# haoyuzhao123/CGRayTracing

Hardware: AMD Instinct MI355X
Metric: Mrays/sec (primary+secondary) at 1920x1080 spp=64 (higher is better)
Workload: dtype f64

## Files before the change

cgraytracing_amd/_capi.py:

```python
from __future__ import annotations

import ctypes as C
import os

import sys

_HERE = os.path.dirname(os.path.abspath(__file__))
CGRT_VERSION = 112
LIB_PATH = os.path.join(_HERE, "libcgrt.so")
if os.environ.get("CGRT_LIB"):
    if os.environ.get("CGRT_DEV_LIBS") == "1":
        LIB_PATH = os.environ["CGRT_LIB"]
        print("cgraytracing_amd: DEVELOPMENT library %s (CGRT_LIB + CGRT_DEV_LIBS=1)" % LIB_PATH, file=sys.stderr)
    else:
        print("cgraytracing_amd: CGRT_LIB ignored (set CGRT_DEV_LIBS=1 to load a development build)", file=sys.stderr)

CGRT_OK = 0
CGRT_NCOUNTERS = 8
CNT_RAYS, CNT_HITPOINTS, CNT_WAVE_ITERS, CNT_NODE_TESTS, CNT_TRI_TESTS = 0, 1, 2, 3, 4


class CgrtError(RuntimeError):
    def __init__(self, code, msg):
        super().__init__("libcgrt error %d: %s" % (code, msg))
# ... 8 lines not shown
class Grid(C.Structure):
    _fields_ = [("width", C.c_int32), ("height", C.c_int32), ("rows", C.c_int32), ("row_offset", C.c_int32),
                ("stripe_rows", C.c_int32), ("stripe_rank", C.c_int32), ("stripe_nranks", C.c_int32),
                ("spp", C.c_int32), ("sample_offset", C.c_int32), ("spp_total", C.c_int32),
                ("max_depth", C.c_int32), ("flags", C.c_int32), ("seed", C.c_uint64)]


GRID_STATS, GRID_ACCUMULATE, GRID_SPLIT_SAMPLES, GRID_NO_REORDER, GRID_FORCE_REORDER, GRID_HITPOINTS = 1, 2, 4, 8, 16, 32
GRID_NO_TILE_ORDER, GRID_DIFFUSE_TILES, GRID_NO_SPHERE_PAIRS, GRID_NO_SPHERE_MASKS = 64, 128, 256, 512
GRID_SAMPLE_RELAY, GRID_NO_SAMPLE_RELAY, GRID_SAMPLE_RELAY_4 = 1024, 2048, 4096
GRID_RELAY_MIRROR, GRID_RELAY_NO_MIRROR = 8192, 16384
GRID_RELAY_CHUNKS_FIRST, GRID_RELAY_MIRROR_FIRST, GRID_RELAY_INTERLEAVED, GRID_RELAY_ORDER_MASK = 32768, 65536, 98304, 98304
GRID_NO_LENS_STAGE, GRID_NO_SURE_TILES = 131072, 262144
GRID_RELAY_COST_START, GRID_NO_RELAY_COST_START, GRID_RELAY_BOOST, GRID_NO_RELAY_BOOST = 524288, 1048576, 2097152, 4194304
GRID_NO_LENS_TABLE, GRID_LENS_TABLE = 8388608, 16777216


class Photons(C.Structure):
    _fields_ = [("light", C.c_double * 3), ("jitter", C.c_double), ("power", C.c_double), ("alpha", C.c_double),
                ("nphotons", C.c_int64), ("hashsize", C.c_int32), ("batch", C.c_int32), ("seed", C.c_uint64),
                ("initial_radius", C.c_double), ("pair_cap", C.c_int64)]


class PpmResult(C.Structure):
    _fields_ = [("image", C.c_void_p), ("rgb8", C.c_void_p), ("hp16", C.c_void_p), ("hp_cap", C.c_uint64),
                ("hp_count", C.c_uint64), ("n_events", C.c_uint64), ("n_pairs", C.c_uint64), ("n_batch_halvings", C.c_uint64),
                ("ms_eye", C.c_double),
                ("ms_table", C.c_double), ("ms_photons", C.c_double), ("ms_gather", C.c_double)]


# ... 58 lines not shown
class RayPixels(C.Structure):
    _fields_ = [("width", C.c_int32), ("rows", C.c_int32), ("spp", C.c_int32), ("pad_", C.c_int32), ("pixel", C.c_void_p)]


class PhotonRays(C.Structure):
    _fields_ = [("n", C.c_int64), ("org3", C.c_void_p), ("dir3", C.c_void_p), ("flux3", C.c_void_p), ("keys", C.c_void_p),
                ("draws", C.c_void_p)]


RAYS_STATS = 1
RAYS_NO_SIGN_PASS = 2
RAYS_HITPOINTS = 4
RAYS_SKIP_TRANSPARENT = 8
STEP_NONE, STEP_HITPOINT, STEP_REFLECT, STEP_SPLIT = 0, 1, 2, 3
PROBE_SQRT, PROBE_NORMALIZED, PROBE_SPHERE_LEN, PROBE_SPHERE_LEN_PAIR = 0, 1, 2, 4

_DP = C.POINTER(C.c_double)
SIGNATURES = {
    "cgrt_version": (C.c_int, []),
    "cgrt_last_error": (C.c_char_p, []),
    "cgrt_scene_create": (C.c_int, [C.POINTER(C.c_void_p)]),
    "cgrt_scene_destroy": (None, [C.c_void_p]),
    "cgrt_scene_set_build": (C.c_int, [C.c_void_p, C.c_int]),
    "cgrt_scene_build_info": (C.c_int, [C.c_void_p, C.POINTER(BuildInfo)]),
    "cgrt_scene_add_sphere": (C.c_int, [C.c_void_p, _DP, C.c_double, _DP, C.c_double, C.c_double]),
    "cgrt_scene_add_texture": (C.c_int, [C.c_void_p, C.c_void_p, C.c_int, C.c_int, _DP, _DP, C.c_double,
                                         C.c_double, C.c_int]),
    "cgrt_scene_add_plane": (C.c_int, [C.c_void_p, _DP, _DP, _DP, C.c_double, C.c_double, C.c_int]),
    "cgrt_scene_add_mesh_file": (C.c_int, [C.c_void_p, C.c_char_p, C.c_double, _DP, _DP, C.c_double, C.c_double,
                                           C.c_int]),
# ... 72 lines not shown
    "cgrt_occlusion_rays_host": (C.c_int, [C.c_void_p, C.POINTER(Rays), C.POINTER(Occlusion), C.c_void_p]),
    "cgrt_occlusion_rays_variant": (C.c_int, [C.c_void_p, C.POINTER(Rays), C.c_char_p, C.c_size_t]),
    "cgrt_bounce_rays": (C.c_int, [C.c_void_p, C.POINTER(Rays), C.POINTER(Bounce), C.c_void_p, C.c_void_p]),
    "cgrt_bounce_rays_host": (C.c_int, [C.c_void_p, C.POINTER(Rays), C.POINTER(Bounce), C.c_void_p]),
    "cgrt_bounce_rays_variant": (C.c_int, [C.c_void_p, C.POINTER(Rays), C.c_char_p, C.c_size_t]),
    "cgrt_wavefront_rays": (C.c_int, [C.c_void_p, C.POINTER(Rays), C.POINTER(Wavefront), C.c_void_p, C.POINTER(C.c_uint64), C.c_void_p]),
    "cgrt_wavefront_rays_host": (C.c_int, [C.c_void_p, C.POINTER(Rays), C.POINTER(Wavefront), C.c_void_p, C.POINTER(C.c_uint64)]),
    "cgrt_wavefront_rays_variant": (C.c_int, [C.c_void_p, C.POINTER(Rays), C.c_char_p, C.c_size_t]),
    "cgrt_scene_last_wavefront": (C.c_int, [C.c_void_p, C.POINTER(C.c_int64), C.POINTER(C.c_int64), C.POINTER(C.c_int32)]),
    "cgrt_scene_last_wavefront_rays": (C.c_int, [C.c_void_p, C.c_void_p]),
    "cgrt_camera_rays": (C.c_int, [C.POINTER(Camera), C.POINTER(Grid), C.c_void_p, C.c_void_p, C.c_void_p, C.c_void_p]),
    "cgrt_camera_rays_host": (C.c_int, [C.POINTER(Camera), C.POINTER(Grid), C.c_void_p, C.c_void_p, C.c_void_p]),
    "cgrt_intersect_rays": (C.c_int, [C.c_void_p, C.c_int, C.c_void_p, C.c_void_p, C.c_void_p, C.c_int,
                                      C.c_void_p, C.c_void_p, C.c_void_p]),
    "cgrt_math_probe": (C.c_int, [C.c_int, C.c_int, C.c_void_p, C.c_int64, C.c_void_p]),
}

_lib = None


def lib():
    global _lib
    if _lib is None:
        if not os.path.exists(LIB_PATH):
            raise ImportError(
                "cgraytracing_amd: %s not found -- build the HIP library first "
                "(make -C cgraytracing_amd/csrc, or __graft_entry__.build()). There is no CPU fallback." % LIB_PATH)
        try:
            import torch
        except ImportError:
# ... 18 lines not shown
```

cgraytracing_amd/csrc/cgrt_build.cpp:

```cpp
#include "cgrt_build.h"

#include <algorithm>
#include <atomic>
#include <chrono>
#include <future>
#include <thread>
#include <unordered_map>
#include <cmath>
#include <cstdio>
#include <cstdlib>
#include <cstring>

namespace cgrt {

namespace {

inline double hi3(double a, double b, double c) { return (a > b && a > c) ? a : (b > c ? b : c); }
inline double lo3(double a, double b, double c) { return (a < b && a < c) ? a : (b < c ? b : c); }
inline float round_down(double v) {
    float f = (float)v;
    return ((double)f > v) ? std::nextafterf(f, -INFINITY) : f;
}
inline float round_up(double v) {
    float f = (float)v;
// ... 987 lines not shown
    d.light_hf_only = plane_trees ? 1 : 0;
    for (const ObjRec &o : objs)
        if (o.kind == KIND_PLANE && o.tree >= 0 && !(o.transp < kEps && trees[(size_t)o.tree].hfield >= 0)) d.light_hf_only = 0;
    d.prun_begin = d.prun_end = 0;
    if (!k.no_plane_run) {
        auto eligible = [&](int j) { return objs[(size_t)j].kind == KIND_PLANE && objs[(size_t)j].axis >= 0 && objs[(size_t)j].tree < 0; };
        int b = 0;
        while (b < d.n_lds && objs[(size_t)b].kind == KIND_PLANE && !eligible(b)) b++;
        int j = b;
        while (j < d.n_lds && eligible(j)) j++;
        if (j - b >= 3) {
            d.prun_begin = b;
            d.prun_end = j;
        }
    }
}

}
```

cgraytracing_amd/csrc/cgrt_eye.hpp:

```cpp
#ifndef CGRT_EYE_HPP
#define CGRT_EYE_HPP
#include "cgrt_lens_stage.h"
#include "cgrt_scene_walk.hpp"
#include "cgrt_sphere_mask.h"
#include "cgrt_sure_first.h"
#include "cgrt_variants.h"

struct Pending {
    V3 o, d, adj;
    int32_t depth_left;
    uint32_t path;
};

#ifndef CGRT_DIFF_WAVES
#define CGRT_DIFF_WAVES 8
#endif
#ifndef CGRT_DIFF_DOF_WAVES
#define CGRT_DIFF_DOF_WAVES 6
#endif
static constexpr int kDiffWaves = CGRT_DIFF_WAVES, kDiffDofWaves = CGRT_DIFF_DOF_WAVES;

__host__ __device__ __forceinline__ void lens_disc(uint64_t k_smp, double &sx, double &sy) {
    uint64_t ctr = k_smp;
    while (true) {
// ... 1293 lines not shown
        out[i] = sqrt_cr(in[i]);
    } else if (op == CGRT_PROBE_NORMALIZED) {
        const V3 v = normalized(ld3(in + 3 * i));
        out[3 * i] = v.x;
        out[3 * i + 1] = v.y;
        out[3 * i + 2] = v.z;
    } else if (op == CGRT_PROBE_SPHERE_LEN) {
        const double *p = in + 10 * i;
        out[i] = sphere_len(ld3(p), p[3], ld3(p + 4), ld3(p + 7));
    } else {
        const double *p = in + 14 * i;
        sphere_len_pair(ld3(p), p[3], ld3(p + 4), p[7], ld3(p + 8), ld3(p + 11), out[2 * i], out[2 * i + 1]);
    }
}

#endif
```

cgraytracing_amd/csrc/cgrt_frame.h:

```cpp
#ifndef CGRT_FRAME_H
#define CGRT_FRAME_H
#include <algorithm>
#include <cmath>
#include <cstddef>
#include <cstdint>
#include <cstdio>
#include <cstdlib>
#include <string>

#include "../../include/cgrt.h"
#include "cgrt_lens_stage.h"
#include "cgrt_relay.h"

struct GridParams {
    int32_t W, H, rows, row_offset, stripe_rows, stripe_rank, stripe_nranks;
    int32_t spp, sample_offset, max_depth;
    int32_t accumulate;
    int32_t xcd_tiles;
    int32_t chunks, chunk_spp;
    double *partial;
    uint32_t *partial_nhit;
    const unsigned char *light;
    int32_t light_mode, tile_order;
    const uint32_t *wmask;
// ... 155 lines not shown
    bool no_sure_tiles = false;
    bool no_order_reuse = false;
    int relay_chunks = kRelayDefaultChunks;
    long long relay_tiles = 0;
    int relay_mirror = -1;
    int relay_order = -1;
    int relay_start = -1;
    int relay_probe_spp = kRelayProbeSpp;
    bool relay_boost_off = false;
    uint32_t relay_boost_num = kRelayBoostNum, relay_boost_den = kRelayBoostDen;
    long long relay_boost_tiles = -1;
    int lens_stage = -1;
    int lens_table = -1;
    long long lens_table_bytes = 0;
    bool lens_table_bytes_set = false;
    const char *timeline_file = nullptr;
};
inline const char *env_str(const char *name) { const char *e = std::getenv(name); return e ? e : ""; }
inline bool env_on(const char *name) { const char *e = env_str(name); return *e && *e != '0'; }
inline int env_positive(const char *name, int def) { const int v = std::atoi(env_str(name)); return v > 0 ? v : def; }
inline int relay_order_named(const char *e) {
    const std::string v(e);
    if (v == "chunks_first" || v == "0") return kRelayChunksFirst;
    if (v == "mirror_first" || v == "1") return kRelayMirrorFirst;
    if (v == "interleaved" || v == "2") return kRelayInterleaved;
    return -1;
}
inline int relay_start_named(const char *e) {
    const std::string v(e);
    if (v == "list" || v == "0") return kRelayStartList;
// ... 59 lines not shown
            std::fprintf(stderr, "cgrt: CGRT_RELAY_START=%s names no start order of this library (list, cost): the default is used\n", env_str("CGRT_RELAY_START"));
        {
            const int ps = std::atoi(env_str("CGRT_RELAY_PROBE_SPP"));
            if (ps == 1 || ps == 2 || ps == 4) k.relay_probe_spp = ps;
        }
        k.lens_stage = lens_stage_named(env_str("CGRT_LENS_STAGE"));
        if (k.lens_stage < 0 && *env_str("CGRT_LENS_STAGE"))
            std::fprintf(stderr, "cgrt: CGRT_LENS_STAGE=%s names no form of this library (off, lds): the default is used\n", env_str("CGRT_LENS_STAGE"));
        k.lens_table = lens_table_named(env_str("CGRT_LENS_TABLE"));
        if (k.lens_table < 0 && *env_str("CGRT_LENS_TABLE"))
            std::fprintf(stderr, "cgrt: CGRT_LENS_TABLE=%s is neither off nor on: the default is used\n", env_str("CGRT_LENS_TABLE"));
        if (*env_str("CGRT_LENS_TABLE_BYTES")) {
            k.lens_table_bytes = std::max(std::atoll(env_str("CGRT_LENS_TABLE_BYTES")), 0ll);
            k.lens_table_bytes_set = true;
        }
        return k;
    }();
    EyeKnobs k = once;
    k.timeline_file = *env_str("CGRT_TIMELINE_FILE") ? env_str("CGRT_TIMELINE_FILE") : nullptr;
    if (!relay_boost_named(env_str("CGRT_RELAY_BOOST"), k.relay_boost_off, k.relay_boost_num, k.relay_boost_den)) {
        static bool said = false;
        if (!said)
            std::fprintf(stderr, "cgrt: CGRT_RELAY_BOOST=%s is neither off nor a threshold num/den (integers, num <= %u, 1 <= den <= %u): the default is used\n",
                         env_str("CGRT_RELAY_BOOST"), kRelayBoostMaxTerm, kRelayBoostMaxTerm);
        said = true;
    }
    if (*env_str("CGRT_RELAY_BOOST_TILES")) k.relay_boost_tiles = std::max(std::atoll(env_str("CGRT_RELAY_BOOST_TILES")), 0ll);
    return k;
}

// ... 284 lines not shown
```

cgraytracing_amd/csrc/cgrt_hip.hip:

```cpp
#include <hip/hip_runtime.h>

#include <algorithm>
#include <atomic>
#include <chrono>
#include <cmath>
#include <cstdio>
#include <cstdlib>
#include <cstring>
#include <exception>
#include <map>
#include <mutex>
#include <string>
#include <type_traits>
#include <vector>

#include "../../include/cgrt.h"
#include "cgrt_build.h"
#include "cgrt_rng.hpp"
#include "cgrt_types.h"

#include "cgrt_device_math.hpp"
#include "cgrt_grid.hpp"
#include "cgrt_traverse.hpp"
#include "cgrt_bezier.hpp"
// ... 605 lines not shown

enum class EyeForm { Image, Sched, SpillSph, SpillGen, Capture, Light, LightHF, Diffuse };
struct EyeLaunch {
    EyeForm form;
    EyeFlags k;
    DeviceScene dev;
    size_t lds;
    const char *what() const {
        static const char *const names[] = {"eye pass", "eye pass", "eye pass, SPILL (spheres)", "eye pass, SPILL (general)",
                                            "Hitpoint capture", "eye pass, light tiles", "eye pass, light tiles (HFONLY)",
                                            "eye pass, diffuse tiles"};
        return form <= EyeForm::Sched && k.bez ? "eye pass (Bezier)" : names[(int)form];
    }
};

static EyeLaunch eye_launch(const cgrt_scene *s, const cgrt_camera *cam, const cgrt_grid *grid, const EyeKnobs &kn, bool capture) {
    const DeviceScene &d = s->dev;
    const bool dof = cam->lens_radius > 0, glass = d.has_glass != 0 && grid->max_depth > 1;
    const bool spill = d.n_objs > d.n_lds;
    EyeLaunch L;
    L.dev = d;
    if (capture || (spill && !d.all_spheres)) {
        L.form = capture ? EyeForm::Capture : EyeForm::SpillGen;
        L.dev = with_resident(d, general_resident(s, dof, capture));
        L.k = general_flags(dof, capture, L.dev.n_objs > L.dev.n_lds);
    } else if (spill) {
        L.form = EyeForm::SpillSph;
        L.k = spill_sph_flags(dof, glass);
    } else {
        const bool bez = d.has_bezier != 0, trees = d.has_mesh != 0 || bez;
        L.k = image_flags(trees, bez, dof, glass, !trees && d.all_spheres != 0,
                          (grid->flags & CGRT_GRID_STATS) != 0 && d.has_mesh != 0 && !bez);
        const bool plain_scene = (d.has_mesh == 0 && d.has_bezier == 0) || d.single_ray != 0;
        const size_t n_wt = (size_t)((grid->width + kWaveTileW - 1) / kWaveTileW) * ((grid->rows + kWaveTileH - 1) / kWaveTileH);
        const bool reorder = grid->spp >= 4 && !(grid->flags & CGRT_GRID_NO_REORDER) && n_wt > 1 && n_wt < (1u << 30) &&
                             (!plain_scene || (grid->flags & CGRT_GRID_FORCE_REORDER) || kn.force_reorder);
        L.form = reorder ? EyeForm::Sched : EyeForm::Image;
        L.k.pair = L.form == EyeForm::Image && L.k.sph && L.k.glass && !L.k.stats && s->order.ok && !(grid->flags & CGRT_GRID_NO_SPHERE_PAIRS);
    }
    L.lds = eye_lds(L.k, L.dev) + (L.form == EyeForm::Image || L.form == EyeForm::Sched ? (size_t)kn.lds_pad : 0);
    return L;
}
static EyeLaunch light_launch(const DeviceScene &d, bool dof, const EyeKnobs &kn) {
    const bool trees = d.light_trees != 0, hf = trees && d.light_hf_only && !kn.no_hfonly;
    EyeLaunch L;
    L.form = hf ? EyeForm::LightHF : EyeForm::Light;
    L.k = light_flags(trees, dof, hf);
    L.dev = d;
    L.lds = eye_lds(L.k, d);
    return L;
}
static EyeLaunch diffuse_launch(const DeviceScene &d, bool dof) {
    EyeLaunch L;
    L.form = EyeForm::Diffuse;
// ... 286 lines not shown
int cgrt_scene_last_inkernel_diffuse_tiles(const cgrt_scene *s, int64_t *n_tiles) {
    NEED_COMMITTED(s, n_tiles);
    ON_DEVICE(s->device);
    return last_class3_tiles(s->order, TileOrderPlan::InKernel, n_tiles);
}
int cgrt_scene_last_lens_stage(const cgrt_scene *s, int64_t *lds_tiles, int64_t *area_tiles) {
    NEED_COMMITTED(s, lds_tiles && area_tiles);
    ON_DEVICE(s->device);
    return last_lens_stage(s->order, lds_tiles, area_tiles);
}
int cgrt_scene_last_lens_table(const cgrt_scene *s, int64_t *entries, int64_t *capacity, int32_t *reused) {
    NEED_COMMITTED(s, entries && capacity && reused);
    ON_DEVICE(s->device);
    return last_lens_table(s->order, s->lens, entries, capacity, reused);
}
int cgrt_scene_last_sample_relay(const cgrt_scene *s, int64_t *tiles, int32_t *chunks, int64_t *parked_values) {
    NEED_COMMITTED(s, tiles && chunks && parked_values);
    ON_DEVICE(s->device);
    return last_sample_relay(s->order, s->relay, tiles, chunks, parked_values);
}
int cgrt_scene_last_relay_form(const cgrt_scene *s, int32_t *mirror, int32_t *order) {
    NEED_COMMITTED(s, mirror && order);
    last_relay_form(s->order, s->relay, mirror, order);
    return CGRT_OK;
}

int cgrt_scene_last_relay_start(const cgrt_scene *s, uint32_t *start, int64_t start_cap, uint32_t *wcost, int64_t cost_cap, int64_t *t,
                                int64_t *n_wave_tiles, int32_t *reused) {
    NEED_COMMITTED(s, t && n_wave_tiles && reused);
    ON_DEVICE(s->device);
// ... 231 lines not shown
    if (n < 0) return fail(CGRT_ERR_INVALID, "cgrt_math_probe: negative n");
    if (n > ((int64_t)1 << 28)) return fail(CGRT_ERR_LIMIT, "cgrt_math_probe: more than 2^28 elements");
    if (n == 0) return CGRT_OK;
    const size_t n_in = op == CGRT_PROBE_SQRT ? 1 : (op == CGRT_PROBE_NORMALIZED ? 3 : (op == CGRT_PROBE_SPHERE_LEN ? 10 : 14)),
                 n_out = op == CGRT_PROBE_NORMALIZED ? 3 : (op == CGRT_PROBE_SPHERE_LEN_PAIR ? 2 : 1);
    ON_DEVICE(device);
    HostStage hs;
    const double *d_in = hs.in(in, (size_t)n * n_in * sizeof(double));
    double *d_out = hs.out(out, (size_t)n * n_out * sizeof(double));
    if (const int rc = hs.error()) return rc;
    hipLaunchKernelGGL(math_probe_kernel, dim3((unsigned)((n + 255) / 256)), dim3(256), 0, 0, op, d_in, (long long)n, d_out);
    HIP_TRY(hipGetLastError());
    return hs.finish(CGRT_OK);
}

}

#include "cgrt_ppm_plan.h"
#include "cgrt_ppm_table.hpp"
#include "cgrt_photon_trace.hpp"
#include "cgrt_ppm_apply.hpp"
#include "cgrt_ppm_session.hpp"
#include "cgrt_output.hpp"

#ifdef CGRT_UTIL
extern "C" void cgrt_util_dump(unsigned long long *out) {
    (void)hipDeviceSynchronize();
    (void)hipMemcpyFromSymbol(out, HIP_SYMBOL(g_util), sizeof(unsigned long long) * 64);
    unsigned long long z[64] = {0};
    (void)hipMemcpyToSymbol(HIP_SYMBOL(g_util), z, sizeof(z));
// ... 3 lines not shown
```

cgraytracing_amd/csrc/cgrt_scene_walk.hpp:

```cpp
#ifndef CGRT_SCENE_WALK_HPP
#define CGRT_SCENE_WALK_HPP
#include "cgrt_bezier.hpp"
#include "cgrt_traverse.hpp"
#include "cgrt_wg_lds.h"

__device__ __forceinline__ bool texture_color(const TexRec &t, const uint8_t *__restrict__ texels, V3 point, V3 &out) {
    V3 d = point - ld3(t.p);
    const V3 n = ld3(t.n);
    d = d - n * dot(d, n);
    const double te = 1e-2;
    const int rows = t.rows, cols = t.cols;
    int r, c;
    if (d.x < te && d.x > -te) {
        if (!(0 < d.y && d.y < t.lenx && 0 < d.z && d.z < t.leny)) return false;
        r = (int)floor(d.y / t.lenx * rows);
        c = (int)floor(d.z / t.leny * cols);
    } else if (d.y < te && d.y > -te) {
        if (!(0 < d.x && d.x < t.lenx && 0 < d.z && d.z < t.leny)) return false;
        c = (int)floor(d.x / t.lenx * cols);
        r = (int)floor(d.z / t.leny * rows);
    } else if (d.z < te && d.z > -te) {
        if (!(0 < d.x && d.x < t.lenx && 0 < d.y && d.y < t.leny)) return false;
        c = (int)floor(d.x / t.lenx * cols);
        r = rows - 1 - (int)floor(d.y / t.leny * rows);
// ... 249 lines not shown
        static_assert(!PAIR || (SPH && !SPILL), "PAIR: the LDS-resident sphere loop");
        static_assert(!MASKED || (SPH && !SPILL && !PAIR && !NRM), "MASKED: the terminal-diffuse body's sphere loop");
        if (MASKED && masked) {
            for (uint32_t m = mask; m != 0u; m &= m - 1u) {
                const int i = __builtin_ctz(m);
                const double len = sphere_len(objs[i], o, d);
                if (len < best.t) {
                    best.t = len;
                    best.id = i;
                }
            }
            return best;
        }
        int i_single = 0;
        if (PAIR) {
            for (int i = 0; i + 1 < n_lds; i += 2) {
                double lenA, lenB;
                const ObjRec &A = objs[i], &B = objs[i + 1];
                sphere_len_pair(ld3(A.a), A.s0, ld3(B.a), B.s0, o, d, lenA, lenB);
                if (lenA < best.t) {
                    best.t = lenA;
                    best.id = i;
                }
                if (lenB < best.t) {
                    best.t = lenB;
                    best.id = i + 1;
                }
            }
            i_single = n_lds & ~1;
        }
// ... 148 lines not shown
```

cgraytracing_amd/csrc/cgrt_types.h:

```cpp
#ifndef CGRT_TYPES_H
#define CGRT_TYPES_H
#include <stddef.h>
#include <stdint.h>

namespace cgrt {

static constexpr double kEps = 1e-4;
static constexpr double kInf = 1e10;
static constexpr int kMinKd = 10;
static constexpr double kBoxPad = 1.001e-4;
static constexpr int kMaxDepth = 5;

enum ObjKind : int32_t { KIND_SPHERE = 0, KIND_PLANE = 1, KIND_MESH = 2, KIND_BEZIER = 3 };

struct ObjRec {
    double a[3];
    double b[3];
    double s0;
    double col[3];
    double refl, transp;
    int32_t kind;
    int32_t tree;
    int32_t tex;
    int32_t aux;
// ... 115 lines not shown
    int32_t prim_obj;
    int32_t has_mesh;
    int32_t has_bezier;
    int32_t all_spheres;
    int32_t has_glass;
    int32_t cached_tree;
    int32_t cached_nodes;
    int32_t has_wide;
    int32_t light_trees;
    int32_t light_ok;
    int32_t n_cover;
    int32_t prim_finish;
    int32_t prun_begin, prun_end;
    int32_t single_ray;
    int32_t light_hf_only;
};

}
#endif
```

cgraytracing_amd/engine.py:

```python
from __future__ import annotations

import ctypes as C
import os
import weakref

import numpy as np

from . import _capi
from ._capi import Camera as _CCamera
from ._capi import Grid as _CGrid
from ._capi import check
from .scene import Camera


def _d3(v):
    return (C.c_double * 3)(*[float(x) for x in v])


_RELAY_ORDERS = ("chunks_first", "mirror_first", "interleaved")
_RELAY_STARTS = ("list", "cost")


def _grid_flags(stats, split_samples, reorder, force_reorder, tile_order, diffuse_tiles, sphere_pairs, sphere_masks, lens_stage, sure_tiles, lens_table=None):
    on = (stats, _capi.GRID_STATS), (split_samples, _capi.GRID_SPLIT_SAMPLES), (force_reorder, _capi.GRID_FORCE_REORDER), (diffuse_tiles, _capi.GRID_DIFFUSE_TILES)
    off = ((reorder, _capi.GRID_NO_REORDER), (tile_order, _capi.GRID_NO_TILE_ORDER), (sphere_pairs, _capi.GRID_NO_SPHERE_PAIRS),
           (sphere_masks, _capi.GRID_NO_SPHERE_MASKS), (lens_stage, _capi.GRID_NO_LENS_STAGE), (sure_tiles, _capi.GRID_NO_SURE_TILES))
    table = 0 if lens_table is None else _capi.GRID_LENS_TABLE if lens_table else _capi.GRID_NO_LENS_TABLE
    return sum(f for v, f in on if v) | sum(f for v, f in off if not v) | table


def _relay_flag(sample_relay, relay_mirror=None, relay_order=None, relay_start=None, relay_boost=None):
    form = 0 if relay_mirror is None else (_capi.GRID_RELAY_MIRROR if relay_mirror else _capi.GRID_RELAY_NO_MIRROR)
    if relay_boost is not None:
        form |= _capi.GRID_RELAY_BOOST if relay_boost else _capi.GRID_NO_RELAY_BOOST
    if relay_start is not None:
        if relay_start not in _RELAY_STARTS:
            raise ValueError("relay_start: None, " + ", ".join(repr(o) for o in _RELAY_STARTS))
        form |= _capi.GRID_RELAY_COST_START if relay_start == "cost" else _capi.GRID_NO_RELAY_COST_START
    if relay_order is not None:
        if relay_order not in _RELAY_ORDERS:
            raise ValueError("relay_order: None, " + ", ".join(repr(o) for o in _RELAY_ORDERS))
# ... 153 lines not shown
        return box[: n.value], ref[: n.value], need.value

    def _structs(self, camera, width, height, rows, spp, max_depth, seed, row_offset, stripe, sample_offset,
                 spp_total, flags):
        camera = camera or Camera()
        cc = _CCamera(_d3(camera.cam), camera.half_width, camera.focus_plane, camera.lens_radius)
        s_rows, s_rank, s_n = stripe if stripe else (0, 0, 1)
        g = _CGrid(width, height, rows, row_offset, s_rows, s_rank, s_n, spp, sample_offset,
                   spp_total if spp_total else spp, max_depth, flags, seed)
        return cc, g

    def trace_grid(self, width, height, spp=1, camera=None, max_depth=5, seed=12345, rows=None, row_offset=0,
                   stripe=None, sample_offset=0, spp_total=None, out=None, nhit=None, counters=None, stream=None,
                   stats=False, accumulate=False, split_samples=False, reorder=True, force_reorder=False, tile_order=True,
                   diffuse_tiles=False, sphere_pairs=True, sphere_masks=True, sample_relay=None,
                   relay_mirror=None, relay_order=None, lens_stage=True, sure_tiles=True, relay_start=None, relay_boost=None, lens_table=None):
        import torch

        rows = height - row_offset if rows is None else rows
        dev = torch.device("cuda", self.device)
        if out is None:
            out = torch.zeros((rows, width, 3), dtype=torch.float32, device=dev)
        if nhit is None:
            nhit = torch.zeros((rows, width), dtype=torch.int32, device=dev)
        elif nhit is False:
            nhit = None
        if counters is None:
            counters = torch.zeros((_capi.CGRT_NCOUNTERS,), dtype=torch.int64, device=dev)
        assert out.is_contiguous() and out.dtype == torch.float32 and tuple(out.shape) == (rows, width, 3)
        cc, g = self._structs(camera, width, height, rows, spp, max_depth, seed, row_offset, stripe, sample_offset,
                              spp_total, (_capi.GRID_ACCUMULATE if accumulate else 0) |
                              _grid_flags(stats, split_samples, reorder, force_reorder, tile_order, diffuse_tiles, sphere_pairs, sphere_masks, lens_stage, sure_tiles, lens_table) |
                              _relay_flag(sample_relay, relay_mirror, relay_order, relay_start, relay_boost))
        st = stream if stream is not None else torch.cuda.current_stream(dev).cuda_stream
        check(self._L.cgrt_trace_grid(self._h, C.byref(cc), C.byref(g), out.data_ptr(),
                                      nhit.data_ptr() if nhit is not None else None,
                                      counters.data_ptr(), C.c_void_p(st)))
        return out, nhit, counters

    _WANT = ("acc", "nhit", "hit")

    def camera_rays(self, width, height, spp=1, camera=None, seed=12345, rows=None, row_offset=0, stripe=None,
                    sample_offset=0, stream=None):
        import torch

        rows = height - row_offset if rows is None else rows
        dev = torch.device("cuda", self.device)
# ... 437 lines not shown
        buf = C.create_string_buffer(160)
        check(self._L.cgrt_wavefront_rays_variant(self._h, C.byref(r), buf, len(buf)))
        return buf.value.decode()

    def rays_variant(self, max_depth=5, want=("acc", "nhit", "hit"), stats=False):
        full = 1 if ("acc" in want or "nhit" in want) else None
        r = _capi.Rays(1, None, None, None, 0, 0, max_depth, _capi.RAYS_STATS if stats else 0)
        o = _capi.RayResults(full, None, 1 if "hit" in want else None, None, None)
        buf = C.create_string_buffer(160)
        check(self._L.cgrt_trace_rays_variant(self._h, C.byref(r), C.byref(o), buf, len(buf)))
        return buf.value.decode()

    def trace_grid_host(self, width, height, spp=1, camera=None, max_depth=5, seed=12345, rows=None, row_offset=0,
                        stripe=None, sample_offset=0, spp_total=None, stats=False, split_samples=False, reorder=True,
                        force_reorder=False, tile_order=True, diffuse_tiles=False, sphere_pairs=True, sphere_masks=True, sample_relay=None,
                        relay_mirror=None, relay_order=None, lens_stage=True, sure_tiles=True, relay_start=None, relay_boost=None, lens_table=None):
        rows = height - row_offset if rows is None else rows
        rgb = np.zeros((rows, width, 3), np.float32)
        nhit = np.zeros((rows, width), np.uint32)
        cnt = np.zeros((_capi.CGRT_NCOUNTERS,), np.uint64)
        cc, g = self._structs(camera, width, height, rows, spp, max_depth, seed, row_offset, stripe, sample_offset,
                              spp_total,
                              _grid_flags(stats, split_samples, reorder, force_reorder, tile_order, diffuse_tiles, sphere_pairs, sphere_masks, lens_stage, sure_tiles, lens_table) |
                              _relay_flag(sample_relay, relay_mirror, relay_order, relay_start, relay_boost))
        check(self._L.cgrt_trace_grid_host(self._h, C.byref(cc), C.byref(g), rgb.ctypes.data, nhit.ctypes.data,
                                           cnt.ctypes.data))
        return dict(rgb=rgb, nhit=nhit, counters=cnt, nrays=int(cnt[_capi.CNT_RAYS]),
                    nhp=int(cnt[_capi.CNT_HITPOINTS]))

    def last_tile_order(self):
        n = C.c_int64()
        check(self._L.cgrt_scene_last_tile_order(self._h, None, None, None, 0, C.byref(n)))
        if n.value == 0:
            return None
        plan, lst, cls = np.zeros(5, np.uint32), np.zeros(n.value, np.uint32), np.zeros(n.value, np.uint8)
        check(self._L.cgrt_scene_last_tile_order(self._h, plan.ctypes.data, lst.ctypes.data, cls.ctypes.data, n.value, C.byref(n)))
        return dict(plan=plan, list=lst, cls=cls)

# ... 2 lines not shown
        check(self._L.cgrt_scene_last_sphere_masks(self._h, None, 0, C.byref(n)))
        if n.value == 0:
            return None
        masks = np.zeros(n.value, np.uint32)
        check(self._L.cgrt_scene_last_sphere_masks(self._h, masks.ctypes.data, n.value, C.byref(n)))
        return masks

    def last_sure_tiles(self):
        n = C.c_int64()
        check(self._L.cgrt_scene_last_sure_tiles(self._h, None, 0, C.byref(n)))
        if n.value == 0:
            return None
        sure = np.zeros(n.value, np.uint8)
        check(self._L.cgrt_scene_last_sure_tiles(self._h, sure.ctypes.data, n.value, C.byref(n)))
        return sure

    def last_tile_order_reused(self):
        f = C.c_int32()
        check(self._L.cgrt_scene_last_tile_order_reused(self._h, C.byref(f)))
        return bool(f.value)

    def last_sample_relay(self):
        t, k, v = C.c_int64(), C.c_int32(), C.c_int64()
        check(self._L.cgrt_scene_last_sample_relay(self._h, C.byref(t), C.byref(k), C.byref(v)))
        return dict(tiles=int(t.value), chunks=int(k.value), parked_values=int(v.value))

    def last_relay_form(self):
        m, o = C.c_int32(), C.c_int32()
        check(self._L.cgrt_scene_last_relay_form(self._h, C.byref(m), C.byref(o)))
        return None if m.value < 0 else dict(mirror=bool(m.value), order=_RELAY_ORDERS[o.value])
# ... 391 lines not shown
```

include/cgrt.h:

```cpp
#ifndef CGRT_H
#define CGRT_H

#include <stddef.h>
#include <stdint.h>

#ifdef __cplusplus
extern "C" {
#endif

#define CGRT_VERSION 112

enum {
    CGRT_OK = 0,
    CGRT_ERR_INVALID = -1,
    CGRT_ERR_IO = -2,
    CGRT_ERR_DEVICE = -3,
    CGRT_ERR_UNSUPPORTED = -4,
    CGRT_ERR_LIMIT = -5
};

typedef struct cgrt_scene cgrt_scene;

typedef struct cgrt_camera {
    double cam[3];
// ... 31 lines not shown
    CGRT_GRID_SAMPLE_RELAY_4 = 4096,
    CGRT_GRID_RELAY_MIRROR = 8192,
    CGRT_GRID_RELAY_NO_MIRROR = 16384,
    CGRT_GRID_RELAY_CHUNKS_FIRST = 32768,
    CGRT_GRID_RELAY_MIRROR_FIRST = 65536,
    CGRT_GRID_RELAY_INTERLEAVED = 98304,
    CGRT_GRID_RELAY_ORDER_MASK = 98304,
    CGRT_GRID_RELAY_COST_START = 524288,
    CGRT_GRID_NO_RELAY_COST_START = 1048576,
    CGRT_GRID_RELAY_BOOST = 2097152,
    CGRT_GRID_NO_RELAY_BOOST = 4194304,
    CGRT_GRID_NO_LENS_STAGE = 131072,
    CGRT_GRID_NO_LENS_TABLE = 8388608,
    CGRT_GRID_LENS_TABLE = 16777216,
    CGRT_GRID_NO_SURE_TILES = 262144,
    CGRT_GRID_HITPOINTS = 32,
    CGRT_GRID_SPLIT_SAMPLES = 4
};

enum {
    CGRT_CNT_RAYS = 0,
    CGRT_CNT_HITPOINTS = 1,
    CGRT_CNT_WAVE_ITERS = 2,
    CGRT_CNT_NODE_TESTS = 3,
    CGRT_CNT_TRI_TESTS = 4,
    CGRT_NCOUNTERS = 8
};

typedef struct cgrt_scene_stats {
    int32_t n_objects, n_spheres, n_planes, n_meshes, n_beziers, n_textures, n_trees, committed;
// ... 253 lines not shown
int cgrt_scene_last_tile_order(const cgrt_scene *s, uint32_t *plan5, uint32_t *list, uint8_t *cls, int64_t cap, int64_t *n_tiles);

int cgrt_scene_last_sphere_masks(const cgrt_scene *s, uint32_t *masks, int64_t cap, int64_t *n_wave_tiles);
int cgrt_scene_last_sure_tiles(const cgrt_scene *s, uint8_t *sure, int64_t cap, int64_t *n_wave_tiles);
int cgrt_scene_last_tile_order_reused(const cgrt_scene *s, int32_t *reused);

int cgrt_trace_grid_diffuse_variant(const cgrt_scene *s, const cgrt_camera *cam, const cgrt_grid *grid, char *name, size_t cap);
int cgrt_scene_last_diffuse_tiles(const cgrt_scene *s, int64_t *n_tiles);
int cgrt_scene_last_inkernel_diffuse_tiles(const cgrt_scene *s, int64_t *n_tiles);
int cgrt_scene_last_sample_relay(const cgrt_scene *s, int64_t *tiles, int32_t *chunks, int64_t *parked_values);
int cgrt_scene_last_relay_form(const cgrt_scene *s, int32_t *mirror, int32_t *order);
int cgrt_scene_last_relay_start(const cgrt_scene *s, uint32_t *start, int64_t start_cap, uint32_t *wcost, int64_t cost_cap, int64_t *t,
                                int64_t *n_wave_tiles, int32_t *reused);
int cgrt_scene_last_lens_stage(const cgrt_scene *s, int64_t *lds_tiles, int64_t *area_tiles);
int cgrt_scene_last_lens_table(const cgrt_scene *s, int64_t *entries, int64_t *capacity, int32_t *reused);

int cgrt_relay_start_host(int32_t k, int32_t chunk_spp, int32_t spp, int64_t cap, int32_t extent, int64_t n01, int64_t n012, int64_t n_tiles,
                          const uint32_t *list, const uint32_t *wcost, int32_t width, int32_t rows, uint32_t *start, int64_t start_cap,
                          int64_t *t);

int cgrt_scene_last_relay_boost(const cgrt_scene *s, int64_t *promoted, int32_t *k_boost, int64_t *boost_cap, uint64_t *cost_sum,
                                int32_t *num, int32_t *den, int32_t *wg_slots, uint32_t *bslot, int64_t slot_cap);
int cgrt_relay_boost_host(int32_t k, int32_t chunk_spp, int32_t spp, int64_t cap, int32_t extent, int64_t n01, int64_t n012, int64_t n_tiles,
                          const uint32_t *list, const uint32_t *wcost, int32_t width, int32_t rows, int32_t k_boost, int32_t boost_chunk_spp,
                          int64_t boost_cap, int32_t num, int32_t den, int32_t wg_slots, uint32_t *start, int64_t start_cap, uint32_t *bslot,
                          int64_t slot_cap, int64_t *t, int64_t *promoted, uint64_t *cost_sum);

int cgrt_lens_samples(uint64_t seed, const int64_t *pixel, const int32_t *sample, int n, double radius, double *out3);

enum { CGRT_PROBE_SQRT = 0, CGRT_PROBE_NORMALIZED = 1, CGRT_PROBE_SPHERE_LEN = 2, CGRT_PROBE_SPHERE_LEN_PAIR = 4  };
int cgrt_math_probe(int device, int op, const double *in, int64_t n, double *out);

#ifdef __cplusplus
}
#endif
#endif
```

Baseline: 111,900.

## Skip distant spheres when whole wave starts inside the single glass sphere

At scene commit it finds the one transparent sphere and computes a conservative mask of the spheres that can overlap it. In the sphere-pair intersection loop, when every active lane's ray origin lies strictly inside that sphere, only the masked spheres are tested and the loop returns early. This targets redundant intersection tests for rays bouncing inside glass. It costs an extra ballot and distance check per call, and it depends on the geometric margin being conservative enough to stay exact.

New measurement: 120,800 (median of 6 runs). +8.0%, better.

```diff
diff --git a/cgraytracing_amd/_capi.py b/cgraytracing_amd/_capi.py
--- a/cgraytracing_amd/_capi.py
+++ b/cgraytracing_amd/_capi.py
@@ -46,6 +46,7 @@
 GRID_NO_LENS_STAGE, GRID_NO_SURE_TILES = 131072, 262144
 GRID_RELAY_COST_START, GRID_NO_RELAY_COST_START, GRID_RELAY_BOOST, GRID_NO_RELAY_BOOST = 524288, 1048576, 2097152, 4194304
 GRID_NO_LENS_TABLE, GRID_LENS_TABLE = 8388608, 16777216
+GRID_NO_INSIDE_TRIPS = 33554432
 
 
 class Photons(C.Structure):
@@ -134,6 +135,7 @@
 RAYS_SKIP_TRANSPARENT = 8
 STEP_NONE, STEP_HITPOINT, STEP_REFLECT, STEP_SPLIT = 0, 1, 2, 3
 PROBE_SQRT, PROBE_NORMALIZED, PROBE_SPHERE_LEN, PROBE_SPHERE_LEN_PAIR = 0, 1, 2, 4
+PROBE_INSIDE_LOOP = 5
 
 _DP = C.POINTER(C.c_double)
 SIGNATURES = {
@@ -236,6 +238,8 @@
     "cgrt_intersect_rays": (C.c_int, [C.c_void_p, C.c_int, C.c_void_p, C.c_void_p, C.c_void_p, C.c_int,
                                       C.c_void_p, C.c_void_p, C.c_void_p]),
     "cgrt_math_probe": (C.c_int, [C.c_int, C.c_int, C.c_void_p, C.c_int64, C.c_void_p]),
+    "cgrt_scene_inside_spheres": (C.c_int, [C.c_void_p, C.c_void_p, C.c_void_p, C.c_void_p, C.c_int32, C.POINTER(C.c_int32)]),
+    "cgrt_inside_probe": (C.c_int, [C.c_void_p, C.c_int, C.c_void_p, C.c_int64, C.c_void_p]),
 }
 
 _lib = None
diff --git a/cgraytracing_amd/csrc/cgrt_build.cpp b/cgraytracing_amd/csrc/cgrt_build.cpp
--- a/cgraytracing_amd/csrc/cgrt_build.cpp
+++ b/cgraytracing_amd/csrc/cgrt_build.cpp
@@ -1025,6 +1025,16 @@
             d.prun_end = j;
         }
     }
-}
-
-}
+    d.inside = InsideTrait{};
+    if (d.all_spheres && d.n_objs == d.n_lds && d.n_objs <= kInsideSpheresMax) {
+        std::vector<InsideBall> balls;
+        std::vector<double> transp;
+        for (const ObjRec &o : objs) {
+            balls.push_back(InsideBall{{o.a[0], o.a[1], o.a[2]}, o.s0});
+            transp.push_back(o.transp);
+        }
+        d.inside = inside_trait(balls.data(), transp.data(), d.n_objs, true);
+    }
+}
+
+}
diff --git a/cgraytracing_amd/csrc/cgrt_eye.hpp b/cgraytracing_amd/csrc/cgrt_eye.hpp
--- a/cgraytracing_amd/csrc/cgrt_eye.hpp
+++ b/cgraytracing_amd/csrc/cgrt_eye.hpp
@@ -1331,4 +1331,27 @@
     }
 }
 
+__global__ void inside_loop_probe_kernel(DeviceScene sc, InsideTrait guarded, const double *__restrict__ in, long long n, double *__restrict__ out) {
+    const long long i = (long long)blockIdx.x * blockDim.x + threadIdx.x;
+    if (i >= n) return;
+    const V3 o = ld3(in + 6 * i), d = ld3(in + 6 * i + 3);
+    RayKey rk{0, 1, false, 0u};
+    LdsAux aux;
+    aux.bl = nullptr;
+    aux.lnodes = nullptr;
+    uint32_t nn = 0, nt = 0;
+    sc.inside = InsideTrait{};
+    const SceneHit a = intersect_scene<false, false, true, false, false, false, false, false, true>(sc.objs, sc.n_lds, sc.n_objs, sc, o, d, rk, true, aux, nn, nt);
+    sc.inside = guarded;
+    const SceneHit b = intersect_scene<false, false, true, false, false, false, false, false, true>(sc.objs, sc.n_lds, sc.n_objs, sc, o, d, rk, true, aux, nn, nt);
+    bool took = false;
+    for (int k = 0; k < kInsideMax && k < guarded.n && !took; k++)
+        took = __ballot(!starts_inside(o, ld3(sc.objs[guarded.idx[k]].a), guarded.rin2[k])) == 0ull;
+    out[5 * i] = a.t;
+    out[5 * i + 1] = (double)a.id;
+    out[5 * i + 2] = b.t;
+    out[5 * i + 3] = (double)b.id;
+    out[5 * i + 4] = took ? 1.0 : 0.0;
+}
+
 #endif
diff --git a/cgraytracing_amd/csrc/cgrt_frame.h b/cgraytracing_amd/csrc/cgrt_frame.h
--- a/cgraytracing_amd/csrc/cgrt_frame.h
+++ b/cgraytracing_amd/csrc/cgrt_frame.h
@@ -193,6 +193,7 @@
     int lens_table = -1;
     long long lens_table_bytes = 0;
     bool lens_table_bytes_set = false;
+    bool no_inside_trips = false;
     const char *timeline_file = nullptr;
 };
 inline const char *env_str(const char *name) { const char *e = std::getenv(name); return e ? e : ""; }
@@ -282,6 +283,12 @@
             k.lens_table_bytes = std::max(std::atoll(env_str("CGRT_LENS_TABLE_BYTES")), 0ll);
             k.lens_table_bytes_set = true;
         }
+        {
+            const std::string v(env_str("CGRT_INSIDE_TRIPS"));
+            k.no_inside_trips = v == "off" || v == "0";
+            if (!v.empty() && !k.no_inside_trips && v != "on" && v != "1")
+                std::fprintf(stderr, "cgrt: CGRT_INSIDE_TRIPS=%s is neither off nor on: the default is used\n", v.c_str());
+        }
         return k;
     }();
     EyeKnobs k = once;
diff --git a/cgraytracing_amd/csrc/cgrt_hip.hip b/cgraytracing_amd/csrc/cgrt_hip.hip
--- a/cgraytracing_amd/csrc/cgrt_hip.hip
+++ b/cgraytracing_amd/csrc/cgrt_hip.hip
@@ -643,6 +643,16 @@
     }
 };
 
+static InsideTrait inside_paying(const DeviceScene &d) {
+    InsideTrait t{};
+    for (int k = 0; k < d.inside.n; k++)
+        if (inside_pays(d.inside, k, d.n_lds)) {
+            t.idx[t.n] = d.inside.idx[k], t.mask[t.n] = d.inside.mask[k], t.rin2[t.n] = d.inside.rin2[k];
+            t.n++;
+        }
+    return t;
+}
+
 static EyeLaunch eye_launch(const cgrt_scene *s, const cgrt_camera *cam, const cgrt_grid *grid, const EyeKnobs &kn, bool capture) {
     const DeviceScene &d = s->dev;
     const bool dof = cam->lens_radius > 0, glass = d.has_glass != 0 && grid->max_depth > 1;
@@ -667,6 +677,8 @@
         L.form = reorder ? EyeForm::Sched : EyeForm::Image;
         L.k.pair = L.form == EyeForm::Image && L.k.sph && L.k.glass && !L.k.stats && s->order.ok && !(grid->flags & CGRT_GRID_NO_SPHERE_PAIRS);
     }
+    L.dev.inside = InsideTrait{};
+    if (L.k.pair && !(grid->flags & CGRT_GRID_NO_INSIDE_TRIPS) && !kn.no_inside_trips) L.dev.inside = inside_paying(d);
     L.lds = eye_lds(L.k, L.dev) + (L.form == EyeForm::Image || L.form == EyeForm::Sched ? (size_t)kn.lds_pad : 0);
     return L;
 }
@@ -983,6 +995,13 @@
     ON_DEVICE(s->device);
     return last_lens_table(s->order, s->lens, entries, capacity, reused);
 }
+int cgrt_scene_inside_spheres(const cgrt_scene *s, int32_t *index, uint32_t *mask, double *rin2, int32_t cap, int32_t *n) {
+    NEED_COMMITTED(s, n && (cap <= 0 || (index && mask && rin2)));
+    const InsideTrait &t = s->dev.inside;
+    *n = t.n;
+    for (int k = 0; k < t.n && k < cap; k++) index[k] = t.idx[k], mask[k] = t.mask[k], rin2[k] = t.rin2[k];
+    return CGRT_OK;
+}
 int cgrt_scene_last_sample_relay(const cgrt_scene *s, int64_t *tiles, int32_t *chunks, int64_t *parked_values) {
     NEED_COMMITTED(s, tiles && chunks && parked_values);
     ON_DEVICE(s->device);
@@ -1244,6 +1263,25 @@
     return hs.finish(CGRT_OK);
 }
 
+int cgrt_inside_probe(const cgrt_scene *s, int op, const double *rays, int64_t n, double *out) {
+    NEED_COMMITTED(s, rays && out);
+    if (op != CGRT_PROBE_INSIDE_LOOP) return fail(CGRT_ERR_INVALID, "cgrt_inside_probe: unknown op");
+    if (n < 0) return fail(CGRT_ERR_INVALID, "cgrt_inside_probe: negative n");
+    if (n > ((int64_t)1 << 28)) return fail(CGRT_ERR_LIMIT, "cgrt_inside_probe: more than 2^28 elements");
+    const DeviceScene &d = s->dev;
+    if (!d.all_spheres || d.n_objs < 1 || d.n_objs != d.n_lds)
+        return fail(CGRT_ERR_UNSUPPORTED, "cgrt_inside_probe: the pair loop serves sphere-only scenes whose list is resident");
+    if (n == 0) return CGRT_OK;
+    ON_DEVICE(s->device);
+    HostStage hs;
+    const double *d_in = hs.in(rays, (size_t)n * 6 * sizeof(double));
+    double *d_out = hs.out(out, (size_t)n * 5 * sizeof(double));
+    if (const int rc = hs.error()) return rc;
+    hipLaunchKernelGGL(inside_loop_probe_kernel, dim3((unsigned)((n + 255) / 256)), dim3(256), 0, 0, d, inside_paying(d), d_in, (long long)n, d_out);
+    HIP_TRY(hipGetLastError());
+    return hs.finish(CGRT_OK);
+}
+
 }
 
 #include "cgrt_ppm_plan.h"
diff --git a/cgraytracing_amd/csrc/cgrt_inside_sphere.h b/cgraytracing_amd/csrc/cgrt_inside_sphere.h
--- /dev/null
+++ b/cgraytracing_amd/csrc/cgrt_inside_sphere.h
@@ -0,0 +1,81 @@
+#ifndef CGRT_INSIDE_SPHERE_H
+#define CGRT_INSIDE_SPHERE_H
+#include <stdint.h>
+#include <cmath>
+
+#if defined(__HIPCC__)
+#define CGRT_INSIDE_HD __host__ __device__ inline __attribute__((always_inline))
+#else
+#define CGRT_INSIDE_HD inline
+#endif
+
+static constexpr int kInsideMax = 1;
+static constexpr int kInsideSpheresMax = 32;
+static constexpr double kInsideRound = 8e-15;
+
+struct InsideBall {
+    double c[3], r2;
+};
+struct InsideTrait {
+    int32_t n;
+    int32_t idx[kInsideMax];
+    uint32_t mask[kInsideMax];
+    double rin2[kInsideMax];
+};
+
+CGRT_INSIDE_HD bool inside_finite(const InsideBall &b) {
+    return fabs(b.c[0]) < 1e150 && fabs(b.c[1]) < 1e150 && fabs(b.c[2]) < 1e150 && b.r2 > 0 && b.r2 < 1e300;
+}
+CGRT_INSIDE_HD double inside_rin2(double r2) {
+    const double r = sqrt(r2), r_in = r * (1 - 1e-9) - 1e-6;
+    return (r2 > 0 && r2 < 1e300 && r_in > 0) ? r_in * r_in : 0.0;
+}
+CGRT_INSIDE_HD double inside_margin(double D, double ri, double rj) {
+    const double Lj = D + ri, S = D + ri + rj;
+    return 2 * (2 * sqrt(kInsideRound * Lj * Lj) + sqrt(kInsideRound * ri * ri)) + (S * 1e-9 + 1e-6);
+}
+CGRT_INSIDE_HD uint32_t inside_full_mask(int n) { return n >= 32 ? 0xffffffffu : (1u << n) - 1u; }
+
+CGRT_INSIDE_HD uint32_t inside_mask(const InsideBall *s, int n, int i) {
+    const uint32_t full = inside_full_mask(n);
+    if (n < 1 || n > kInsideSpheresMax || i < 0 || i >= n) return full;
+    for (int j = 0; j < n; j++)
+        if (!inside_finite(s[j])) return full;
+    if (!(inside_rin2(s[i].r2) > 0)) return full;
+    const double ri = sqrt(s[i].r2);
+    uint32_t mask = 1u << i;
+    for (int j = 0; j < n; j++) {
+        if (j == i) continue;
+        const double dx = s[j].c[0] - s[i].c[0], dy = s[j].c[1] - s[i].c[1], dz = s[j].c[2] - s[i].c[2];
+        const double D = sqrt(dx * dx + dy * dy + dz * dz), rj = sqrt(s[j].r2);
+        if (!(D > ri + rj + inside_margin(D, ri, rj))) mask |= 1u << j;
+    }
+    return mask;
+}
+
+template <class V> CGRT_INSIDE_HD bool starts_inside(V o, V c, double rin2) {
+    const double lx = c.x - o.x, ly = c.y - o.y, lz = c.z - o.z;
+    return lx * lx + ly * ly + lz * lz < rin2;
+}
+
+inline InsideTrait inside_trait(const InsideBall *s, const double *transp, int n, bool all_spheres) {
+    InsideTrait t{};
+    if (!all_spheres || n < 1 || n > kInsideSpheresMax) return t;
+    int count = 0;
+    for (int j = 0; j < n; j++)
+        if (!(transp[j] < 1e-4)) count++;
+    if (count > kInsideMax) return t;
+    for (int j = 0; j < n; j++)
+        if (!(transp[j] < 1e-4)) {
+            t.idx[t.n] = j;
+            t.mask[t.n] = inside_mask(s, n, j);
+            t.rin2[t.n] = t.mask[t.n] == inside_full_mask(n) ? 0.0 : inside_rin2(s[j].r2);
+            t.n++;
+        }
+    return t;
+}
+inline bool inside_pays(const InsideTrait &t, int k, int n) {
+    return k < t.n && t.rin2[k] > 0 && 5 * (int)__builtin_popcount(t.mask[k]) <= 4 * n;
+}
+
+#endif
diff --git a/cgraytracing_amd/csrc/cgrt_scene_walk.hpp b/cgraytracing_amd/csrc/cgrt_scene_walk.hpp
--- a/cgraytracing_amd/csrc/cgrt_scene_walk.hpp
+++ b/cgraytracing_amd/csrc/cgrt_scene_walk.hpp
@@ -287,6 +287,19 @@
         }
         int i_single = 0;
         if (PAIR) {
+            for (int k = 0; k < kInsideMax && k < sc.inside.n; k++) {
+                const bool in = starts_inside(o, ld3(objs[sc.inside.idx[k]].a), sc.inside.rin2[k]);
+                if (__ballot(on && !in) != 0ull) continue;
+                for (uint32_t m = sc.inside.mask[k]; m != 0u; m &= m - 1u) {
+                    const int i = __builtin_ctz(m);
+                    const double len = sphere_len(objs[i], o, d);
+                    if (len < best.t) {
+                        best.t = len;
+                        best.id = i;
+                    }
+                }
+                return best;
+            }
             for (int i = 0; i + 1 < n_lds; i += 2) {
                 double lenA, lenB;
                 const ObjRec &A = objs[i], &B = objs[i + 1];
diff --git a/cgraytracing_amd/csrc/cgrt_types.h b/cgraytracing_amd/csrc/cgrt_types.h
--- a/cgraytracing_amd/csrc/cgrt_types.h
+++ b/cgraytracing_amd/csrc/cgrt_types.h
@@ -2,6 +2,8 @@
 #define CGRT_TYPES_H
 #include <stddef.h>
 #include <stdint.h>
+
+#include "cgrt_inside_sphere.h"
 
 namespace cgrt {
 
@@ -153,6 +155,7 @@
     int32_t prun_begin, prun_end;
     int32_t single_ray;
     int32_t light_hf_only;
+    InsideTrait inside;
 };
 
 }
diff --git a/cgraytracing_amd/engine.py b/cgraytracing_amd/engine.py
--- a/cgraytracing_amd/engine.py
+++ b/cgraytracing_amd/engine.py
@@ -21,10 +21,11 @@
 _RELAY_STARTS = ("list", "cost")
 
 
-def _grid_flags(stats, split_samples, reorder, force_reorder, tile_order, diffuse_tiles, sphere_pairs, sphere_masks, lens_stage, sure_tiles, lens_table=None):
+def _grid_flags(stats, split_samples, reorder, force_reorder, tile_order, diffuse_tiles, sphere_pairs, sphere_masks, lens_stage, sure_tiles, lens_table=None, inside_trips=True):
     on = (stats, _capi.GRID_STATS), (split_samples, _capi.GRID_SPLIT_SAMPLES), (force_reorder, _capi.GRID_FORCE_REORDER), (diffuse_tiles, _capi.GRID_DIFFUSE_TILES)
     off = ((reorder, _capi.GRID_NO_REORDER), (tile_order, _capi.GRID_NO_TILE_ORDER), (sphere_pairs, _capi.GRID_NO_SPHERE_PAIRS),
-           (sphere_masks, _capi.GRID_NO_SPHERE_MASKS), (lens_stage, _capi.GRID_NO_LENS_STAGE), (sure_tiles, _capi.GRID_NO_SURE_TILES))
+           (sphere_masks, _capi.GRID_NO_SPHERE_MASKS), (lens_stage, _capi.GRID_NO_LENS_STAGE), (sure_tiles, _capi.GRID_NO_SURE_TILES),
+           (inside_trips, _capi.GRID_NO_INSIDE_TRIPS))
     table = 0 if lens_table is None else _capi.GRID_LENS_TABLE if lens_table else _capi.GRID_NO_LENS_TABLE
     return sum(f for v, f in on if v) | sum(f for v, f in off if not v) | table
 
@@ -208,7 +209,8 @@
                    stripe=None, sample_offset=0, spp_total=None, out=None, nhit=None, counters=None, stream=None,
                    stats=False, accumulate=False, split_samples=False, reorder=True, force_reorder=False, tile_order=True,
                    diffuse_tiles=False, sphere_pairs=True, sphere_masks=True, sample_relay=None,
-                   relay_mirror=None, relay_order=None, lens_stage=True, sure_tiles=True, relay_start=None, relay_boost=None, lens_table=None):
+                   relay_mirror=None, relay_order=None, lens_stage=True, sure_tiles=True, relay_start=None, relay_boost=None, lens_table=None,
+                   inside_trips=True):
         import torch
 
         rows = height - row_offset if rows is None else rows
@@ -224,7 +226,7 @@
         assert out.is_contiguous() and out.dtype == torch.float32 and tuple(out.shape) == (rows, width, 3)
         cc, g = self._structs(camera, width, height, rows, spp, max_depth, seed, row_offset, stripe, sample_offset,
                               spp_total, (_capi.GRID_ACCUMULATE if accumulate else 0) |
-                              _grid_flags(stats, split_samples, reorder, force_reorder, tile_order, diffuse_tiles, sphere_pairs, sphere_masks, lens_stage, sure_tiles, lens_table) |
+                              _grid_flags(stats, split_samples, reorder, force_reorder, tile_order, diffuse_tiles, sphere_pairs, sphere_masks, lens_stage, sure_tiles, lens_table, inside_trips) |
                               _relay_flag(sample_relay, relay_mirror, relay_order, relay_start, relay_boost))
         st = stream if stream is not None else torch.cuda.current_stream(dev).cuda_stream
         check(self._L.cgrt_trace_grid(self._h, C.byref(cc), C.byref(g), out.data_ptr(),
@@ -692,14 +694,15 @@
     def trace_grid_host(self, width, height, spp=1, camera=None, max_depth=5, seed=12345, rows=None, row_offset=0,
                         stripe=None, sample_offset=0, spp_total=None, stats=False, split_samples=False, reorder=True,
                         force_reorder=False, tile_order=True, diffuse_tiles=False, sphere_pairs=True, sphere_masks=True, sample_relay=None,
-                        relay_mirror=None, relay_order=None, lens_stage=True, sure_tiles=True, relay_start=None, relay_boost=None, lens_table=None):
+                        relay_mirror=None, relay_order=None, lens_stage=True, sure_tiles=True, relay_start=None, relay_boost=None, lens_table=None,
+                   inside_trips=True):
         rows = height - row_offset if rows is None else rows
         rgb = np.zeros((rows, width, 3), np.float32)
         nhit = np.zeros((rows, width), np.uint32)
         cnt = np.zeros((_capi.CGRT_NCOUNTERS,), np.uint64)
         cc, g = self._structs(camera, width, height, rows, spp, max_depth, seed, row_offset, stripe, sample_offset,
                               spp_total,
-                              _grid_flags(stats, split_samples, reorder, force_reorder, tile_order, diffuse_tiles, sphere_pairs, sphere_masks, lens_stage, sure_tiles, lens_table) |
+                              _grid_flags(stats, split_samples, reorder, force_reorder, tile_order, diffuse_tiles, sphere_pairs, sphere_masks, lens_stage, sure_tiles, lens_table, inside_trips) |
                               _relay_flag(sample_relay, relay_mirror, relay_order, relay_start, relay_boost))
         check(self._L.cgrt_trace_grid_host(self._h, C.byref(cc), C.byref(g), rgb.ctypes.data, nhit.ctypes.data,
                                            cnt.ctypes.data))
@@ -732,6 +735,20 @@
         sure = np.zeros(n.value, np.uint8)
         check(self._L.cgrt_scene_last_sure_tiles(self._h, sure.ctypes.data, n.value, C.byref(n)))
         return sure
+
+    def inside_spheres(self):
+        n = C.c_int32()
+        check(self._L.cgrt_scene_inside_spheres(self._h, None, None, None, 0, C.byref(n)))
+        idx, mask, rin2 = np.zeros(max(n.value, 1), np.int32), np.zeros(max(n.value, 1), np.uint32), np.zeros(max(n.value, 1), np.float64)
+        check(self._L.cgrt_scene_inside_spheres(self._h, idx.ctypes.data, mask.ctypes.data, rin2.ctypes.data, n.value, C.byref(n)))
+        return [dict(index=int(idx[k]), mask=int(mask[k]), rin2=float(rin2[k])) for k in range(n.value)]
+
+    def inside_probe(self, rays):
+        rays = np.ascontiguousarray(rays, np.float64)
+        assert rays.ndim == 2 and rays.shape[1] == 6
+        out = np.zeros((rays.shape[0], 5), np.float64)
+        check(self._L.cgrt_inside_probe(self._h, _capi.PROBE_INSIDE_LOOP, rays.ctypes.data, rays.shape[0], out.ctypes.data))
+        return out
 
     def last_tile_order_reused(self):
         f = C.c_int32()
diff --git a/include/cgrt.h b/include/cgrt.h
--- a/include/cgrt.h
+++ b/include/cgrt.h
@@ -69,6 +69,7 @@
     CGRT_GRID_NO_LENS_TABLE = 8388608,
     CGRT_GRID_LENS_TABLE = 16777216,
     CGRT_GRID_NO_SURE_TILES = 262144,
+    CGRT_GRID_NO_INSIDE_TRIPS = 33554432,
     CGRT_GRID_HITPOINTS = 32,
     CGRT_GRID_SPLIT_SAMPLES = 4
 };
@@ -352,6 +353,7 @@
                                 int64_t *n_wave_tiles, int32_t *reused);
 int cgrt_scene_last_lens_stage(const cgrt_scene *s, int64_t *lds_tiles, int64_t *area_tiles);
 int cgrt_scene_last_lens_table(const cgrt_scene *s, int64_t *entries, int64_t *capacity, int32_t *reused);
+int cgrt_scene_inside_spheres(const cgrt_scene *s, int32_t *index, uint32_t *mask, double *rin2, int32_t cap, int32_t *n);
 
 int cgrt_relay_start_host(int32_t k, int32_t chunk_spp, int32_t spp, int64_t cap, int32_t extent, int64_t n01, int64_t n012, int64_t n_tiles,
                           const uint32_t *list, const uint32_t *wcost, int32_t width, int32_t rows, uint32_t *start, int64_t start_cap,
@@ -368,6 +370,8 @@
 
 enum { CGRT_PROBE_SQRT = 0, CGRT_PROBE_NORMALIZED = 1, CGRT_PROBE_SPHERE_LEN = 2, CGRT_PROBE_SPHERE_LEN_PAIR = 4  };
 int cgrt_math_probe(int device, int op, const double *in, int64_t n, double *out);
+enum { CGRT_PROBE_INSIDE_LOOP = 5 };
+int cgrt_inside_probe(const cgrt_scene *s, int op, const double *rays, int64_t n, double *out);
 
 #ifdef __cplusplus
 }
```
